# robertvoy/ComfyUI-Distributed

Hardware: NVIDIA H100
Metric: megapixels/sec (higher is better)
Workload: dtype u8

## Files before the change

comfyui-distributed_b200/_native.py:

```python
from __future__ import annotations

import ctypes
import os
from ctypes import POINTER, c_char_p, c_float, c_int, c_int32, c_int64, c_uint32, c_void_p

import numpy as np

HERE = os.path.dirname(os.path.abspath(__file__))
LIB_PATH = os.path.join(HERE, "libusdu_b200.so")

ABI_VERSION = 8
TILE_WORDS = 24
T_X1, T_Y1, T_EW, T_EH, T_PW, T_PH, T_MASK_OFF, T_MASK_PITCH = range(8)
T_TAB_CROP_H, T_TAB_CROP_V, T_TAB_BLEND_H, T_TAB_BLEND_V = 8, 9, 10, 11
T_SUP_X0, T_SUP_Y0, T_SUP_X1, T_SUP_Y1 = 12, 13, 14, 15
T_FULL_X0, T_FULL_Y0, T_FULL_X1, T_FULL_Y1 = 16, 17, 18, 19
TAB_HEADER = 8
PACKED_ROW = 8
FLAG_FAST = 1
FLAG_MMA = 2
FLAG_MMA_KS2 = 4
FLAG_REMOTE_CANVAS = 1 << 24
FILTER_LANCZOS, FILTER_BICUBIC = 0, 1
CROP_ITEM_WORDS = 6
BLEND_ITEM_WORDS = 4
COVER_WORDS = 4
MASK_WORDS = 16
BLOCK_W = 64
BLOCK_H = 32
FAST_BLOCK_W = 128
FAST_BLOCK_H = 32
FAST_TAPS = 7
JOB_WORDS = 32
(J_SRC_A, J_SRC_B, J_LEAD, J_COLS, J_ROWS, J_IX0, J_IY0, J_ROWS_H, J_OX_BASE, J_N_OUT_H, J_ROWS_V, J_OY_BASE, J_N_OUT_V,
 J_DST_X, J_DST_Y, J_OFF_LO, J_OFF_HI, J_ROWS_OUT, J_COLS_OUT, J_CX0, J_CX1, J_CY0, J_CY1, J_FLAGS, J_MPITCH, J_PITCH,
 J_FRAME_LO, J_FRAME_HI, J_NEXT, J_TAPS_H, J_TAPS_V) = range(31)
J_SLOT = 31


class NativeError(RuntimeError):
    pass


_lib = None

_SIGNATURES = {
    "usdu_abi_version": (c_int, []),
    "usdu_last_error": (c_char_p, []),
    "usdu_device_count": (c_int, []),
    "usdu_sm_count": (c_int, []),
    "usdu_resample_ksize": (c_int, [c_int, c_int]),
    "usdu_resample_table_words": (c_int64, [c_int, c_int]),
    "usdu_build_resample_table": (c_int, [c_int, c_int, POINTER(c_int32)]),
    "usdu_build_identity_table": (c_int, [c_int, POINTER(c_int32)]),
    "usdu_filter_ksize": (c_int, [c_int, c_int, c_int]),
    "usdu_filter_table_words": (c_int64, [c_int, c_int, c_int]),
    "usdu_build_filter_table": (c_int, [c_int, c_int, c_int, POINTER(c_int32)]),
    "usdu_nearest_index": (c_int, [c_int, c_int, POINTER(c_int32)]),
    "usdu_table_input_span": (c_int, [POINTER(c_int32), c_int, c_int, POINTER(c_int), POINTER(c_int)]),
    "usdu_box_blur_params": (c_int, [c_float, POINTER(c_int32), POINTER(c_uint32), POINTER(c_uint32)]),
    "usdu_quantize_canvas": (c_int, [c_void_p, c_void_p, c_int, c_int, c_int, c_int64, c_void_p]),
    "usdu_dequantize_canvas": (c_int, [c_void_p, c_void_p, c_int, c_int, c_int, c_int64, c_void_p]),
    "usdu_gather_dequantize": (c_int, [c_void_p, c_void_p, c_int, c_void_p, c_int, c_int, c_int, c_int64, c_void_p]),
    "usdu_level_blend_crop": (c_int, [c_void_p, c_int, c_int, c_int, c_int64, c_void_p, c_void_p, c_void_p, c_int, c_int, c_int, c_void_p, c_int,
                                      c_void_p, c_int, c_int, c_int, c_void_p, c_void_p, c_int, c_void_p, c_int, c_void_p]),
    "usdu_gather_canvas": (c_int, [c_void_p, c_void_p, c_int, c_void_p, c_int, c_int, c_int, c_int64, c_void_p]),
    "usdu_tile_crop_resize_f32": (c_int, [c_void_p, c_int, c_int, c_int, c_void_p, c_void_p, c_int, c_int, c_int, c_void_p, c_int, c_void_p]),
    "usdu_quantize_rows": (c_int, [c_void_p, c_void_p, c_int, c_int, c_int, c_int64, c_int, c_int, c_void_p]),
    "usdu_dequantize_rows": (c_int, [c_void_p, c_void_p, c_int, c_int, c_int, c_int64, c_int, c_int, c_void_p]),
    "usdu_pack_tiles_u8": (c_int, [c_void_p, c_void_p, c_int64, c_void_p]),
    "usdu_unpack_tiles_f32": (c_int, [c_void_p, c_void_p, c_int64, c_void_p]),
    "usdu_t0_denoise": (c_int, [c_void_p, c_void_p, c_void_p, c_int64, c_int64, c_float, c_void_p]),
    "usdu_mask_scratch_bytes": (c_int64, [POINTER(c_int32), c_int]),
    "usdu_build_feather_masks": (c_int, [POINTER(c_int32), c_int, c_void_p, c_void_p, c_void_p]),
    "usdu_plane_resample_u8": (c_int, [c_void_p, c_int, c_int, c_int, c_int64, c_int64, c_void_p, c_int, c_int,
                                       c_void_p, c_int, c_int, c_int, c_int, c_void_p, c_void_p, c_int64, c_int64,
                                       c_void_p]),
    "usdu_plane_pad_fill_u8": (c_int, [c_void_p, c_int, c_int, c_int, c_int64, c_int64, c_int, c_int, c_void_p,
                                       c_void_p, c_void_p, c_int64, c_int64, c_void_p]),
    "usdu_tile_crop_resize": (c_int, [c_void_p, c_int, c_int, c_int, c_int64, c_void_p, c_void_p, c_void_p,
                                      c_int, c_int, c_int, c_void_p, c_int, c_void_p]),
    "usdu_tile_blend": (c_int, [c_void_p, c_int, c_int, c_int, c_int64, c_void_p, c_void_p, c_void_p, c_void_p,
                                c_int, c_void_p, c_int, c_int, c_void_p, c_int, c_int, c_void_p]),
# ... 14 lines not shown
    try:
        h = ctypes.CDLL(LIB_PATH)
    except OSError as e:
        raise NativeError(f"cannot load {LIB_PATH}: {e}") from e
    for name, (res, args) in _SIGNATURES.items():
        try:
            fn = getattr(h, name)
        except AttributeError as e:
            raise NativeError(f"{LIB_PATH} does not export {name}") from e
        fn.restype = res
        fn.argtypes = args
    if h.usdu_abi_version() != ABI_VERSION:
        raise NativeError(f"ABI mismatch: library {h.usdu_abi_version()} != binding {ABI_VERSION}")
    _lib = h
    return h


def _check(status: int, what: str):
    if status != 0:
        msg = lib().usdu_last_error()
        raise NativeError(f"{what} failed ({status}): {msg.decode() if msg else '?'}")


def _i32p(a: np.ndarray):
    assert a.dtype == np.int32 and a.flags["C_CONTIGUOUS"]
    return a.ctypes.data_as(POINTER(c_int32))


def sm_count() -> int:
    n = lib().usdu_sm_count()
    return n if n > 0 else 0


def build_resample_table(in_size: int, out_size: int) -> np.ndarray:
    L = lib()
    words = L.usdu_resample_table_words(in_size, out_size)
    if words < 0:
        _check(int(words), "usdu_resample_table_words")
    tab = np.zeros(int(words), dtype=np.int32)
    _check(L.usdu_build_resample_table(in_size, out_size, _i32p(tab)), "usdu_build_resample_table")
    if tab[4]:
        tab = tab[: int(tab[4]) + out_size * int(tab[6])]
    return np.ascontiguousarray(tab)


def build_filter_table(filt: int, in_size: int, out_size: int) -> np.ndarray:
    L = lib()
    words = L.usdu_filter_table_words(filt, in_size, out_size)
    if words < 0:
        _check(int(words), "usdu_filter_table_words")
    tab = np.zeros(int(words), dtype=np.int32)
    _check(L.usdu_build_filter_table(filt, in_size, out_size, _i32p(tab)), "usdu_build_filter_table")
    return np.ascontiguousarray(tab[: TAB_HEADER + out_size * (2 + int(tab[2]))])


def nearest_index(in_size: int, out_size: int) -> np.ndarray:
    idx = np.zeros(out_size, dtype=np.int32)
    _check(lib().usdu_nearest_index(in_size, out_size, _i32p(idx)), "usdu_nearest_index")
    return idx


def table_input_span(table: np.ndarray, first_out: int, n_out: int):
    a, b = c_int(), c_int()
    _check(lib().usdu_table_input_span(_i32p(table), first_out, n_out, ctypes.byref(a), ctypes.byref(b)),
           "usdu_table_input_span")
    return a.value, b.value
# ... 105 lines not shown
```

comfyui-distributed_b200/csrc/usdu_kernels.cu:

```cuda
#include "usdu_common.cuh"

namespace usdu {

__global__ void __launch_bounds__(kThreads)
quantize_canvas_kernel(const float* __restrict__ img, uint8_t* __restrict__ canvas, int rows, int W3,
                       int64_t pitch, int vec_ok, int H, int y0, int n_rows) {
    const int chunks = (W3 + 15) >> 4;
    const int64_t total = (int64_t)rows * chunks;
    for (int64_t i = (int64_t)blockIdx.x * blockDim.x + threadIdx.x; i < total;
         i += (int64_t)gridDim.x * blockDim.x) {
        const int64_t lrow = i / chunks;
        const int j0 = (int)(i - lrow * chunks) << 4;
        const int64_t fb = lrow / n_rows;
        const int64_t row = fb * H + y0 + (lrow - fb * n_rows);
        const float* src = img + row * W3 + j0;
        uint8_t* dst = canvas + row * pitch + j0;
        if (vec_ok && j0 + 16 <= W3) {
            const float4* s4 = reinterpret_cast<const float4*>(src);
            float4 a = __ldcs(s4), b = __ldcs(s4 + 1), c = __ldcs(s4 + 2), d = __ldcs(s4 + 3);
            uint4 o;
            o.x = quant_u8(a.x) | (quant_u8(a.y) << 8) | (quant_u8(a.z) << 16) | (quant_u8(a.w) << 24);
            o.y = quant_u8(b.x) | (quant_u8(b.y) << 8) | (quant_u8(b.z) << 16) | (quant_u8(b.w) << 24);
            o.z = quant_u8(c.x) | (quant_u8(c.y) << 8) | (quant_u8(c.z) << 16) | (quant_u8(c.w) << 24);
            o.w = quant_u8(d.x) | (quant_u8(d.y) << 8) | (quant_u8(d.z) << 16) | (quant_u8(d.w) << 24);
// ... 415 lines not shown
    const int64_t cap = (int64_t)grid_sms() * 16;
    return (int)(blocks < 1 ? 1 : (blocks > cap ? cap : blocks));
}

static int smem_optin(const void* fn, size_t bytes) {
    if (bytes > 227 * 1024) {
        set_error("kernel needs %zu bytes of shared memory (> 227 KB): patch too large", bytes);
        return USDU_ERR_UNSUPPORTED;
    }
    if (bytes > 48 * 1024) USDU_CUDA(cudaFuncSetAttribute(fn, cudaFuncAttributeMaxDynamicSharedMemorySize, (int)bytes));
    return USDU_OK;
}

}

namespace usdu { namespace fast {
int launch_crop(const uint8_t* canvas, int B, int H, int W, int64_t pitch, const int32_t* tiles, const int32_t* tabs,
                const int32_t* items, int n_items, int patch_w, int patch_h, float* out, cudaStream_t st);
int launch_blend(uint8_t* canvas, int B, int H, int W, int64_t pitch, const int32_t* tiles, const int32_t* tabs,
                 const uint8_t* mask_pool, const int32_t* items, int n_items, const int32_t* cover, int patch_w,
                 int patch_h, const void* src, int src_is_u8, int block_rows, int remote, cudaStream_t st);
} }

namespace usdu { namespace mma {
int launch_crop(const void* canvas, int src_f32, int B, int H, int W, int64_t pitch, const int32_t* tabs, const int32_t* items,
                int n_items, int patch_w, int patch_h, float* out, int two_ksteps, cudaStream_t st);
int launch_blend(uint8_t* canvas, int B, int H, int W, int64_t pitch, const int32_t* tabs, const uint8_t* mask_pool,
                 const int32_t* items, int n_items, int patch_w, int patch_h, const void* src, int src_is_u8, int block_rows,
                 int two_ksteps, cudaStream_t st);
int launch_level(uint8_t* canvas, int B, int H, int W, int64_t pitch, const int32_t* tabs, const uint8_t* mask_pool,
                 const int32_t* bjobs, int n_bheads, int b_patch_w, int b_patch_h, const float* src, int block_rows,
                 const int32_t* cjobs, int n_cjobs, int c_patch_w, int c_patch_h, float* out, const int32_t* expect, int n_slots,
                 int* sync, int two_ksteps, cudaStream_t st);
} }

using namespace usdu;

extern "C" {

int usdu_quantize_rows(const float* img_dev, uint8_t* canvas_dev, int B, int H, int W, int64_t pitch, int y0, int y1,
                       void* stream) {
    USDU_REQUIRE(img_dev && canvas_dev, "usdu_quantize_rows: null pointer");
    USDU_REQUIRE(B > 0 && H > 0 && W > 0, "usdu_quantize_rows: bad shape %dx%dx%d", B, H, W);
    USDU_REQUIRE(0 <= y0 && y0 <= y1 && y1 <= H, "usdu_quantize_rows: bad row range [%d, %d) of %d", y0, y1, H);
    USDU_REQUIRE(pitch >= 3LL * W && pitch % 16 == 0, "usdu_quantize_rows: pitch %lld must be >= 3*W and a multiple of 16", (long long)pitch);
    if (y1 == y0) return USDU_OK;
    const int W3 = W * 3;
    const int vec_ok = (W3 % 4 == 0) && (((uintptr_t)img_dev & 15) == 0) && (((uintptr_t)canvas_dev & 15) == 0);
    const int64_t total = (int64_t)B * (y1 - y0) * ((W3 + 15) / 16);
    const int64_t qblocks = (total + kThreads - 1) / kThreads;
    const int64_t qcap = (int64_t)grid_sms() * 128;
    const int grid = (int)(qblocks < 1 ? 1 : (qblocks > qcap ? qcap : qblocks));
    quantize_canvas_kernel<<<grid, kThreads, 0, (cudaStream_t)stream>>>(img_dev, canvas_dev, B * (y1 - y0), W3, pitch, vec_ok, H, y0, y1 - y0);
    USDU_CUDA(cudaGetLastError());
    return USDU_OK;
}

int usdu_quantize_canvas(const float* img_dev, uint8_t* canvas_dev, int B, int H, int W, int64_t pitch,
                         void* stream) {
    USDU_REQUIRE(H > 0, "usdu_quantize_canvas: bad shape %dx%dx%d", B, H, W);
    return usdu_quantize_rows(img_dev, canvas_dev, B, H, W, pitch, 0, H, stream);
}

int usdu_dequantize_rows(const uint8_t* canvas_dev, float* img_dev, int B, int H, int W, int64_t pitch, int y0, int y1,
                         void* stream) {
    USDU_REQUIRE(img_dev && canvas_dev, "usdu_dequantize_rows: null pointer");
// ... 214 lines not shown
    if (blk_h <= 0 || blk_h > BH) blk_h = BH;
    if (blk_w <= 0 || blk_w > BW) blk_w = BW;
    crop_resize_kernel<<<dim3(n_items, B), kThreads, smem, (cudaStream_t)stream>>>(
        canvas_dev, H, W, pitch, tiles_dev, tabs_dev, items_dev, out_dev, in_pitch, patch_h, blk_w, blk_h);
    USDU_CUDA(cudaGetLastError());
    return USDU_OK;
}

int usdu_tile_crop_resize_f32(const float* image_dev, int B, int H, int W, const int32_t* tabs_dev, const int32_t* items_dev,
                              int n_items, int patch_w, int patch_h, float* out_dev, int flags, void* stream) {
    USDU_REQUIRE(image_dev && tabs_dev && items_dev && out_dev, "usdu_tile_crop_resize_f32: null pointer");
    USDU_REQUIRE(B > 0 && H > 0 && W > 0 && n_items >= 0 && B <= 65535, "usdu_tile_crop_resize_f32: bad shape");
    USDU_REQUIRE(flags & USDU_FLAG_MMA, "usdu_tile_crop_resize_f32: tensor-core job records only (USDU_FLAG_MMA)");
    if (n_items == 0) return USDU_OK;
    return mma::launch_crop(image_dev, 1, B, H, W, (int64_t)W * 3, tabs_dev, items_dev, n_items, patch_w, patch_h, out_dev,
                            (flags & USDU_FLAG_MMA_KS2) ? 1 : 0, (cudaStream_t)stream);
}

int usdu_level_blend_crop(uint8_t* canvas_dev, int B, int H, int W, int64_t pitch, const int32_t* tabs_dev,
                          const uint8_t* mask_pool_dev, const int32_t* bjobs_dev, int n_bheads, int b_patch_w, int b_patch_h,
                          const float* src_dev, int block_rows, const int32_t* cjobs_dev, int n_cjobs, int c_patch_w, int c_patch_h,
                          float* out_dev, const int32_t* expect_dev, int n_slots, int32_t* sync_dev, int flags, void* stream) {
    USDU_REQUIRE(canvas_dev && tabs_dev && mask_pool_dev && bjobs_dev && src_dev && cjobs_dev && out_dev && expect_dev && sync_dev,
                 "usdu_level_blend_crop: null pointer");
    USDU_REQUIRE(B > 0 && B <= 65535 && H > 0 && W > 0 && n_bheads > 0 && n_cjobs > 0 && n_slots > 0, "usdu_level_blend_crop: bad shape");
    USDU_REQUIRE(pitch >= 3LL * W && pitch % 16 == 0, "usdu_level_blend_crop: pitch must be >= 3*W and a multiple of 16");
    USDU_REQUIRE(((uintptr_t)src_dev & 15) == 0, "usdu_level_blend_crop: src must be 16-byte aligned");
    USDU_REQUIRE(flags & USDU_FLAG_MMA, "usdu_level_blend_crop: tensor-core job records only (USDU_FLAG_MMA)");
    return mma::launch_level(canvas_dev, B, H, W, pitch, tabs_dev, mask_pool_dev, bjobs_dev, n_bheads, b_patch_w, b_patch_h, src_dev,
                             block_rows, cjobs_dev, n_cjobs, c_patch_w, c_patch_h, out_dev, expect_dev, n_slots, sync_dev,
                             (flags & USDU_FLAG_MMA_KS2) ? 1 : 0, (cudaStream_t)stream);
}

int usdu_tile_blend(uint8_t* canvas_dev, int B, int H, int W, int64_t pitch, const int32_t* tiles_dev,
                    const int32_t* tabs_dev, const uint8_t* mask_pool_dev, const int32_t* items_dev,
                    int n_items, const int32_t* cover_dev, int patch_w, int patch_h, const void* src_dev,
                    int src_is_u8, int flags, void* stream) {
    USDU_REQUIRE(canvas_dev && tiles_dev && mask_pool_dev && items_dev && src_dev && (cover_dev || (flags & (USDU_FLAG_FAST | USDU_FLAG_MMA))),
                 "usdu_tile_blend: null pointer");
    USDU_REQUIRE(B > 0 && H > 0 && W > 0 && n_items >= 0, "usdu_tile_blend: bad shape");
    USDU_REQUIRE(B <= 65535, "usdu_tile_blend: batch %d exceeds grid.y limit", B);
    USDU_REQUIRE(patch_w > 0 && patch_h > 0, "usdu_tile_blend: patch capacity must be positive");
    if (n_items == 0) return USDU_OK;
    USDU_REQUIRE(pitch >= 3LL * W && pitch % 16 == 0, "usdu_tile_blend: pitch must be >= 3*W and a multiple of 16");
    if (flags & USDU_FLAG_MMA) {
        USDU_REQUIRE(tabs_dev != nullptr, "usdu_tile_blend: tensor-core path needs tables");
        USDU_REQUIRE(((uintptr_t)src_dev & 15) == 0, "usdu_tile_blend: src must be 16-byte aligned");
        return mma::launch_blend(canvas_dev, B, H, W, pitch, tabs_dev, mask_pool_dev, items_dev, n_items, patch_w, patch_h, src_dev,
                                 src_is_u8, (flags >> 8) & 0xFF, (flags & USDU_FLAG_MMA_KS2) ? 1 : 0, (cudaStream_t)stream);
    }
    if (flags & USDU_FLAG_FAST) {
        USDU_REQUIRE(tabs_dev != nullptr, "usdu_tile_blend: fast path needs tables");
        USDU_REQUIRE(((uintptr_t)src_dev & 15) == 0, "usdu_tile_blend: src must be 16-byte aligned");
        return fast::launch_blend(canvas_dev, B, H, W, pitch, tiles_dev, tabs_dev, mask_pool_dev, items_dev, n_items,
                                  cover_dev, patch_w, patch_h, src_dev, src_is_u8, (flags >> 8) & 0xFF,
                                  (flags & USDU_FLAG_REMOTE_CANVAS) ? 1 : 0, (cudaStream_t)stream);
    }
    const int in_pitch = (patch_w * 3 + 15) / 16 * 16;
    const size_t smem = (size_t)BH * BW * 3 + (size_t)patch_h * BW * 3 + (size_t)patch_h * in_pitch;
    const void* fn = src_is_u8 ? (const void*)blend_kernel<true> : (const void*)blend_kernel<false>;
    int s = smem_optin(fn, smem);
    if (s != USDU_OK) return s;
    int blk_h = (flags >> 8) & 0xFF, blk_w = (flags >> 16) & 0xFF;
    if (blk_h <= 0 || blk_h > BH) blk_h = BH;
    if (blk_w <= 0 || blk_w > BW) blk_w = BW;
    if (src_is_u8)
// ... 11 lines not shown
```

comfyui-distributed_b200/csrc/usdu_mma.cu:

```cuda
#include "usdu_common.cuh"
#include "usdu_tma.cuh"
#include <string.h>

namespace usdu {
namespace mma {

constexpr int kT = 256;
constexpr int kOccSmall = 3, kOccLarge = 4;
constexpr int kLargeGridPerSM = 8;
constexpr int BWX = USDU_FAST_BLOCK_W;
constexpr int MIDP = 440;
constexpr int kDBox = BWX * 3 / 2;
constexpr int kBoxB = 256, kBoxR = 48;

__host__ __device__ inline int plane_pitch(int patch_w) { return (patch_w + 31) / 32 * 32 + 16; }
__host__ __device__ inline size_t planes_bytes(int patch_w, int plane_rows) { return (size_t)3 * plane_rows * plane_pitch(patch_w); }
__host__ __device__ inline size_t mid_bytes(int mid_rows) { return (size_t)(mid_rows / 4) * MIDP * 4; }
constexpr size_t kHeadBytes = USDU_JOB_WORDS * 4;

struct JobView {
    const int32_t* j;
    __device__ __forceinline__ int operator[](int i) const { return j[i]; }
    __device__ __forceinline__ int64_t i64(int lo) const { return (int64_t)(uint32_t)j[lo] | ((int64_t)j[lo + 1] << 32); }
};

__device__ __forceinline__ void load_job(int32_t* job_sm, const int32_t* __restrict__ jobs, int idx) {
    if (threadIdx.x < USDU_JOB_WORDS / 4)
        reinterpret_cast<int4*>(job_sm)[threadIdx.x] = __ldg(reinterpret_cast<const int4*>(jobs + (size_t)idx * USDU_JOB_WORDS) + threadIdx.x);
}

__device__ __forceinline__ void mma_uu(int (&d)[4], const uint32_t (&a)[4], uint32_t b0, uint32_t b1) {
    asm("mma.sync.aligned.m16n8k32.row.col.s32.u8.u8.s32 {%0,%1,%2,%3}, {%4,%5,%6,%7}, {%8,%9}, {%0,%1,%2,%3};"
        : "+r"(d[0]), "+r"(d[1]), "+r"(d[2]), "+r"(d[3]) : "r"(a[0]), "r"(a[1]), "r"(a[2]), "r"(a[3]), "r"(b0), "r"(b1));
}
__device__ __forceinline__ void mma_su(int (&d)[4], const uint32_t (&a)[4], uint32_t b0, uint32_t b1) {
    asm("mma.sync.aligned.m16n8k32.row.col.s32.s8.u8.s32 {%0,%1,%2,%3}, {%4,%5,%6,%7}, {%8,%9}, {%0,%1,%2,%3};"
        : "+r"(d[0]), "+r"(d[1]), "+r"(d[2]), "+r"(d[3]) : "r"(a[0]), "r"(a[1]), "r"(a[2]), "r"(a[3]), "r"(b0), "r"(b1));
}

__device__ __forceinline__ int combine(int l0, int l1, int l2) {
    return (l0 + (l1 << 8) + (l2 << 16)) >> kPrecisionBits;
}
// ... 300 lines not shown
            tma::load_3d(raw, &cmap, x, y, b, bar);
            if (two) tma::load_3d(raw + kBoxR * kBoxB, &cmap, x + kBoxB, y, b, bar);
        }
        tma::mbar_wait(bar, 0);
        stage_raw(planes, PB, plane_rows, raw, J[USDU_J_ROWS], J[USDU_J_COLS], sa3 & 15);
    } else if (kSrc == 2) {
        const float* src = reinterpret_cast<const float*>(canvas) + ((int64_t)b * H + J[USDU_J_SRC_B]) * pitch + sa3;
        stage_f32(planes, PB, plane_rows, src, pitch, J[USDU_J_ROWS], J[USDU_J_COLS]);
    } else {
        const uint8_t* src = canvas + ((int64_t)b * H + J[USDU_J_SRC_B]) * pitch + sa3;
        stage_u8(planes, PB, plane_rows, src, pitch, J[USDU_J_ROWS], J[USDU_J_COLS]);
    }
    __syncthreads();
    CropEpilogue epi;
    epi.row_pitch = J[USDU_J_PITCH];
    epi.dst = out + J.i64(USDU_J_OFF_LO) + (int64_t)b * J.i64(USDU_J_FRAME_LO) + (int64_t)J[USDU_J_DST_Y] * epi.row_pitch +
              (int64_t)J[USDU_J_DST_X] * 3;
    epi.ow3 = J[USDU_J_COLS_OUT] * 3;
    epi.rows_out = J[USDU_J_ROWS_OUT];
    both_passes<KSMAX>(planes, mid, tabs, J, PB, plane_rows, J[USDU_J_CY1], epi);
}

struct DTile {
    uint8_t* base;
    int bh;
    __device__ __forceinline__ int strip_off(int strip) const {
        return 4 * strip + (strip >= kDBox / 4 ? bh * kDBox - kDBox : 0);
    }
};

struct BlendOpaque {
    DTile d;
    int nrows;
    uint8_t* rp[2];
    struct Pre {};
    __device__ __forceinline__ void rows(int r0, int r1) {
        rp[0] = (r0 >= 0 && r0 < nrows) ? d.base + r0 * kDBox : nullptr;
        rp[1] = (r1 >= 0 && r1 < nrows) ? d.base + r1 * kDBox : nullptr;
    }
    __device__ __forceinline__ Pre prefetch(int) const { return Pre{}; }
    __device__ __forceinline__ void store(const Pre&, int h, int strip, uint32_t v) {
        if (rp[h] != nullptr) *reinterpret_cast<uint32_t*>(rp[h] + d.strip_off(strip)) = v;
    }
};

struct BlendFeather {
    DTile d;
    const uint8_t* mask;
    int mpitch;
    int cx0, cx1, cy0, cy1;
    uint8_t* rp[2];
    const uint8_t* mp[2];
    struct Pre {
        uint32_t aa[2], ab[2];
        int split;
    };
    __device__ __forceinline__ void rows(int r0, int r1) {
        const bool in0 = r0 >= cy0 && r0 < cy1, in1 = r1 >= cy0 && r1 < cy1;
        rp[0] = in0 ? d.base + r0 * kDBox : nullptr;
        rp[1] = in1 ? d.base + r1 * kDBox : nullptr;
        mp[0] = mask + (int64_t)r0 * mpitch;
        mp[1] = mask + (int64_t)r1 * mpitch;
    }
    __device__ __forceinline__ Pre prefetch(int strip) const {
        const int col = 4 * strip;
        const int pa = col / 3, pb = (col + 3) / 3;
        const bool ina = pa >= cx0 && pa < cx1, inb = pb >= cx0 && pb < cx1;
        Pre p;
        p.split = 3 * pb - col;
#pragma unroll
        for (int h = 0; h < 2; ++h) {
            p.aa[h] = (rp[h] != nullptr && ina) ? (uint32_t)__ldg(mp[h] + pa) : 0u;
            p.ab[h] = (rp[h] != nullptr && inb) ? (uint32_t)__ldg(mp[h] + pb) : 0u;
        }
        return p;
    }
    __device__ __forceinline__ void store(const Pre& p, int h, int strip, uint32_t v) {
        const uint32_t aa = p.aa[h], ab = p.ab[h];
        if ((aa | ab) == 0u) return;
        uint32_t* w = reinterpret_cast<uint32_t*>(rp[h] + d.strip_off(strip));
        if ((aa & ab) == 255u) { *w = v; return; }
        const uint32_t dv = *w;
        uint32_t o = 0;
#pragma unroll
        for (int i = 0; i < 4; ++i) {
            const uint32_t a = i < p.split ? aa : ab;
            o |= composite8((v >> (8 * i)) & 0xFF, (dv >> (8 * i)) & 0xFF, a) << (8 * i);
        }
        *w = o;
    }
};

template <bool kSrcU8, int KSMAX>
__global__ void __launch_bounds__(kT, kOccSmall)
blend_mma_kernel(const int32_t* __restrict__ tabs, const uint8_t* __restrict__ mask_pool, const int32_t* __restrict__ jobs,
                 const void* __restrict__ src_v, int W3, int patch_w, int plane_rows, int mid_rows, int block_rows,
                 const __grid_constant__ CUtensorMap cmap) {
    extern __shared__ __align__(128) uint8_t smem[];
    const size_t dbytes = (size_t)2 * block_rows * kDBox;
    int32_t* job_sm = reinterpret_cast<int32_t*>(smem + dbytes);
    uint64_t* bar = reinterpret_cast<uint64_t*>(smem + dbytes + kHeadBytes);
    uint32_t* mid = reinterpret_cast<uint32_t*>(smem + dbytes + kHeadBytes + 16);
    uint8_t* planes = smem + dbytes + kHeadBytes + 16 + mid_bytes(mid_rows);
    const int PB = plane_pitch(patch_w);
    const int b = blockIdx.y;
    const JobView J{job_sm};
    DTile D{smem, block_rows};
    int idx = blockIdx.x;
    pdl_launch_dependents();
    load_job(job_sm, jobs, idx);
    if (threadIdx.x == 0) tma::mbar_init(bar, 1);
    __syncthreads();
    pdl_wait();
// ... 184 lines not shown
                  (int64_t)J[USDU_J_DST_X] * 3;
        epi.ow3 = J[USDU_J_COLS_OUT] * 3;
        epi.rows_out = J[USDU_J_ROWS_OUT];
        both_passes<KSMAX>(planes, mid, a.tabs, J, PB, a.c_plane_rows, J[USDU_J_CY1], epi);
    }
    __syncthreads();
    if (threadIdx.x == 0) {
        __threadfence();
        s_item = atomicAdd(a.sync + 1, 1);
    }
    __syncthreads();
    if (s_item == total - 1) {
        const int n = 3 + a.n_slots * a.B;
        for (int i = threadIdx.x; i < n; i += kT)
            if (i != 2) a.sync[i] = 0;
        __threadfence();
    }
}

static size_t crop_smem(int patch_w, int plane_rows, int mid_rows, bool use_tma) {
    const size_t region = use_tma ? max(mid_bytes(mid_rows), (size_t)2 * kBoxR * kBoxB) : mid_bytes(mid_rows);
    return region + kHeadBytes + 16 + planes_bytes(patch_w, plane_rows);
}
static size_t blend_smem(int patch_w, int plane_rows, int mid_rows, int block_rows) {
    return (size_t)2 * block_rows * kDBox + kHeadBytes + 16 + planes_bytes(patch_w, plane_rows) + mid_bytes(mid_rows);
}

static int optin(const void* fn, size_t bytes) {
    if (bytes > 227 * 1024) {
        set_error("tensor-core kernel needs %zu bytes of shared memory (> 227 KB)", bytes);
        return USDU_ERR_UNSUPPORTED;
    }
    if (bytes > 48 * 1024) USDU_CUDA(cudaFuncSetAttribute(fn, cudaFuncAttributeMaxDynamicSharedMemorySize, (int)bytes));
    return USDU_OK;
}

static int split_patch_h(int patch_h, int* plane_rows, int* mid_rows, const char* who) {
    *plane_rows = patch_h & 0xFFFF;
    *mid_rows = (patch_h >> 16) & 0xFFFF;
    if (*plane_rows <= 0 || *plane_rows % 8 || *mid_rows < *plane_rows || *mid_rows % 4) {
        set_error("%s: with USDU_FLAG_MMA patch_h carries plane rows (x8) in bits 0..15 and intermediate rows (x4, >= plane rows) "
                  "in bits 16..31; got %d / %d", who, *plane_rows, *mid_rows);
        return USDU_ERR_INVALID;
    }
    return USDU_OK;
}

template <class K, class... Args>
static int launch_one(K kernel, size_t smem, dim3 grid, cudaStream_t st, Args... args) {
    int s = optin((const void*)kernel, smem);
    if (s != USDU_OK) return s;
    USDU_CUDA(launch_pdl(kernel, grid, dim3(kT), smem, st, args...));
    USDU_CUDA(cudaGetLastError());
    return USDU_OK;
}

int launch_crop(const void* canvas, int src_f32, int B, int H, int W, int64_t pitch, const int32_t* tabs, const int32_t* items,
                int n_items, int patch_w, int patch_h, float* out, int two_ksteps, cudaStream_t st) {
    int plane_rows, mid_rows;
    int s = split_patch_h(patch_h, &plane_rows, &mid_rows, "usdu_tile_crop_resize");
    if (s != USDU_OK) return s;
    CUtensorMap cmap;
    memset(&cmap, 0, sizeof(cmap));
    const uint8_t* cv = static_cast<const uint8_t*>(canvas);
    const dim3 grid(n_items, B);
    const int W3 = W * 3;
    const bool large = (int64_t)n_items * B >= (int64_t)kLargeGridPerSM * grid_sms() && !two_ksteps;
#define USDU_CROP_LAUNCH(SRC)                                                                                                                   \
    (two_ksteps ? launch_one(crop_mma_kernel<SRC, 2, kOccSmall>, smem, grid, st, cv, H, pitch, tabs, items, out, patch_w, plane_rows, mid_rows, W3, cmap) \
     : large    ? launch_one(crop_mma_kernel<SRC, 1, kOccLarge>, smem, grid, st, cv, H, pitch, tabs, items, out, patch_w, plane_rows, mid_rows, W3, cmap) \
                : launch_one(crop_mma_kernel<SRC, 1, kOccSmall>, smem, grid, st, cv, H, pitch, tabs, items, out, patch_w, plane_rows, mid_rows, W3, cmap))
    if (src_f32) {
        if (W % 4 != 0 || ((uintptr_t)canvas & 15) != 0) {
            set_error("usdu_tile_crop_resize_f32: the image width must be a multiple of 4 and the image 16-byte aligned");
            return USDU_ERR_UNSUPPORTED;
        }
        const size_t smem = crop_smem(patch_w, plane_rows, mid_rows, false);
        return USDU_CROP_LAUNCH(2);
    }
    bool use_tma = plane_rows <= kBoxR && 12 + patch_w * 3 <= 2 * kBoxB && ((uintptr_t)canvas & 15) == 0;
    if (use_tma) use_tma = tma::encode_u8_3d(&cmap, canvas, (uint64_t)W * 3, (uint64_t)H, (uint64_t)B, (uint64_t)pitch, kBoxB, kBoxR);
    const size_t smem = crop_smem(patch_w, plane_rows, mid_rows, use_tma);
    if (use_tma) return USDU_CROP_LAUNCH(1);
    return USDU_CROP_LAUNCH(0);
#undef USDU_CROP_LAUNCH
}

int launch_blend(uint8_t* canvas, int B, int H, int W, int64_t pitch, const int32_t* tabs, const uint8_t* mask_pool,
                 const int32_t* items, int n_items, int patch_w, int patch_h, const void* src, int src_is_u8, int block_rows,
                 int two_ksteps, cudaStream_t st) {
    if (block_rows != 16 && block_rows != 32) {
        set_error("usdu_tile_blend: the tensor-core path needs a block height of 16 or 32 in flags bits 8..15, got %d", block_rows);
        return USDU_ERR_INVALID;
    }
    int plane_rows, mid_rows;
    int s = split_patch_h(patch_h, &plane_rows, &mid_rows, "usdu_tile_blend");
    if (s != USDU_OK) return s;
    CUtensorMap cmap;
    memset(&cmap, 0, sizeof(cmap));
    if (((uintptr_t)canvas & 15) != 0 ||
// ... 48 lines not shown
```

comfyui-distributed_b200/planner.py:

```python
from __future__ import annotations

import math
import os
from dataclasses import dataclass, field
from typing import Dict, List, Optional, Sequence, Tuple

import numpy as np

from . import _native as nat
from .lru import LruCache


def round_to_multiple(value: int, multiple: int = 8) -> int:
    return round(value / multiple) * multiple


def tile_origins(W: int, H: int, tw: int, th: int) -> List[Tuple[int, int]]:
    cols, rows = math.ceil(W / tw), math.ceil(H / th)
    return [(c * tw, r * th) for r in range(rows) for c in range(cols)]


def _grow(lo: int, hi: int, limit: int, target: int) -> Tuple[int, int]:
    hi = min(hi + (target - (hi - lo)) // 2, limit)
    lo = max(lo - (target - (hi - lo)), 0)
    hi = min(hi + (target - (hi - lo)), limit)
    return lo, hi


@dataclass(frozen=True)
class Tile:
    idx: int
    x: int
    y: int
    x1: int
    y1: int
    x2: int
    y2: int
    pw: int
# ... 355 lines not shown
        best = None
        for k in range(1, world):
            asg = [[] for _ in range(world)]
            for t in self.tiles:
                asg[((t.idx % cols) + k * (t.idx // cols)) % world].append(t.idx)
            if self.conflict_free(asg):
                spread = max(len(a) for a in asg) - min(len(a) for a in asg)
                if best is None or spread < best[0]:
                    best = (spread, asg)
        if best is not None:
            return best[1]
        asg = [[] for _ in range(world)]
        for t in self.tiles:
            asg[t.idx % world].append(t.idx)
        return asg

    def slot_offsets(self, tile_ids: Sequence[int], B: int) -> Tuple[np.ndarray, int]:
        offs = np.zeros(len(tile_ids), dtype=np.int64)
        cur = 0
        for i, tid in enumerate(tile_ids):
            t = self.tiles[tid]
            offs[i] = cur
            cur += B * t.ph * t.pw * 3
        return offs, cur

    def _span_max(self, n_in: int, n_out: int, block: int, aligned: bool) -> int:
        sp = self._tab_span[(n_in, n_out)]
        starts = np.arange(0, n_out, block) if aligned else np.arange(0, n_out)
        ends = np.minimum(starts + block, n_out) - 1
        return int((sp[ends, 1] - sp[starts, 0]).max())

    CTAS_PER_SM = 4
    DEFAULT_SMS = 132

    @classmethod
    def resident_slots(cls) -> int:
        return (nat.sm_count() or cls.DEFAULT_SMS) * cls.CTAS_PER_SM

    def block_shape(self, use_fast: bool, extents: Optional[Sequence[Tuple[int, int]]] = None, frames: int = 1,
                    share: int = 1, mma: bool = False) -> Tuple[int, int]:
        if not use_fast:
            return self._generic_block
        bw = nat.FAST_BLOCK_W
        if not extents:
            return bw, nat.FAST_BLOCK_H
        best = None
        slots = self.resident_slots()
        forced = os.environ.get("USDU_MMA_BH") if mma else None
        for bh in (((int(forced),) if forced else (16, 32)) if mma else (8, 12, 16, 20, 24, 28, 32)):
            n = sum(((w + bw - 1) // bw + 1) * ((h + bh - 1) // bh + 1) for w, h in extents) * frames
            cost = math.ceil(n / max(slots // max(share, 1), 1)) * (bh + 12)
            if best is None or cost < best[0] or (cost == best[0] and bh > best[1]):
                best = (cost, bh)
        return bw, best[1]

    @property
    def _generic_block(self) -> Tuple[int, int]:
        if self._gblock is None:
            bw, bh = nat.BLOCK_W, nat.BLOCK_H
            while True:
                pw_ = max([self._span_max(a, b, bw, False) for (a, b) in self._tab_span] or [bw])
                ph_ = max([self._span_max(a, b, bh, False) for (a, b) in self._tab_span] or [bh])
                smem = nat.BLOCK_H * nat.BLOCK_W * 3 + ph_ * nat.BLOCK_W * 3 + ph_ * ((pw_ * 3 + 15) // 16 * 16)
                if smem <= 200 * 1024 or (bw <= 4 and bh <= 4):
                    break
                if pw_ * bh >= ph_ * bw and bw > 4 or bh <= 4:
                    bw //= 2
                else:
                    bh //= 2
            self._gblock = (bw, bh)
        return self._gblock

    def _crop_block_rows(self, t: Tile, use_fast: bool, bh_max: int) -> int:
        if not use_fast:
            return self._generic_block[1]
        for bh in range(bh_max, 7, -1):
            if self._span_max(t.eh, t.ph, bh, True) <= 40:
                return bh
        return 8

    def kernel_path(self, use_fast=None) -> int:
        path = 2 if use_fast is None else int(use_fast)
        if path >= 2 and not self.mma:
            path = 1
        if path >= 1 and not self.fast:
            path = 0
        return path

    def _mma_crop_rows(self, t: Tile, bh_max: int) -> int:
        key = (t.eh, t.ph)
        for bh in ((32, 16) if bh_max >= 32 else (16,)):
            k0, end, ks = self._tab_k0[key], self._tab_end[key], self._tab_ks[key]
            worst = 0
            for oy0 in range(0, t.ph, bh):
                mv0, mv1 = oy0 // MMA_M, (min(oy0 + bh, t.ph) - 1) // MMA_M
                worst = max(worst, int(end[MMA_M * mv0:min(MMA_M * (mv1 + 1), t.ph)].max() - k0[mv0]))
            if worst <= 48:
                return bh
        return 16

    def crop_worklist(self, tile_ids: Sequence[int], B: int, use_fast: Optional[bool] = None,
                      share: int = 1) -> Tuple[WorkList, np.ndarray, int]:
        path = self.kernel_path(use_fast)
        use_fast = path >= 1
        offs, total = self.slot_offsets(tile_ids, B)
        rows = []
        pw_max = ph_max = 1
        nbytes = 0
        bw, bh_max = self.block_shape(use_fast, [(self.tiles[t].pw - nat.FAST_BLOCK_W, self.tiles[t].ph) for t in tile_ids], B, share,
                                      mma=path == 2)
        for i, tid in enumerate(tile_ids):
            t = self.tiles[tid]
            bh = self._mma_crop_rows(t, bh_max) if path == 2 else self._crop_block_rows(t, use_fast, bh_max)
            ox = np.arange(0, t.pw, bw, dtype=np.int64)
            oy = np.arange(0, t.ph, bh, dtype=np.int64)
            gx, gy = np.meshgrid(ox, oy)
            n = gx.size
            it = np.zeros((n, nat.CROP_ITEM_WORDS), dtype=np.int64)
            it[:, 0], it[:, 1], it[:, 2] = tid, gx.ravel(), gy.ravel()
            it[:, 3], it[:, 4], it[:, 5] = offs[i] & 0xFFFFFFFF, offs[i] >> 32, bh
            rows.append(it)
            pw_max = max(pw_max, self._span_max(t.ew, t.pw, bw, True))
            ph_max = max(ph_max, self._span_max(t.eh, t.ph, bh, True))
            nbytes += t.ew * t.eh * 3 + t.pw * t.ph * 3 * 4
        items = np.concatenate(rows, 0) if rows else np.zeros((0, nat.CROP_ITEM_WORDS), dtype=np.int64)
        if path == 2 and items.shape[0]:
            items, pw_max, ph_max = self._crop_jobs_mma(items)
        elif use_fast and items.shape[0]:
            items = self._crop_jobs(items)
        items = items.astype(np.uint32).view(np.int32) if items.size else items.astype(np.int32)
        ks2 = bool(path == 2 and items.size and (items.reshape(-1, nat.JOB_WORDS)[:, [nat.J_TAPS_H, nat.J_TAPS_V]] > 1).any())
        return WorkList(np.ascontiguousarray(items), None, pw_max, ph_max, nbytes,
                        block_rows=0 if use_fast else bh_max, block_cols=0 if use_fast else bw, path=path, ks2=ks2), offs, total

    def crop_split(self, wl: WorkList, prev_ids: Sequence[int]) -> np.ndarray:
        J = wl.items.reshape(-1, nat.JOB_WORDS).astype(np.int64)
        x0, y0 = J[:, nat.J_SRC_A], J[:, nat.J_SRC_B]
        x1, y1 = x0 + J[:, nat.J_LEAD] + J[:, nat.J_COLS], y0 + J[:, nat.J_ROWS]
        late = np.zeros(J.shape[0], dtype=bool)
        for tid in prev_ids:
            t = self.tiles[tid]
            sx0, sy0, sx1, sy1 = self.support(t)
            if sx1 > sx0 and sy1 > sy0:
# ... 127 lines not shown
            ix1[m] = np.minimum(self._first(key, ox0[m] + nat.FAST_BLOCK_W - 1) + self._tab_taps[key], key[0])
            rows_h[m], taps_h[m] = self._tab_packed[key], self._tab_job_taps[key]
        for key in {(int(a), int(b)) for a, b in zip(eh, ph)}:
            m = (eh == key[0]) & (ph == key[1])
            iy0[m] = self._first(key, oy0[m])
            iy1[m] = np.minimum(self._first(key, oy0[m] + bh[m] - 1) + self._tab_taps[key], key[0])
            rows_v[m], taps_v[m] = self._tab_packed[key], self._tab_job_taps[key]
        J[:, nat.J_TAPS_H], J[:, nat.J_TAPS_V] = taps_h, taps_v
        px_abs = x1 + ix0
        lead = px_abs & 3
        J[:, nat.J_SRC_A], J[:, nat.J_SRC_B], J[:, nat.J_LEAD] = px_abs - lead, y1 + iy0, lead
        J[:, nat.J_COLS], J[:, nat.J_ROWS], J[:, nat.J_IX0], J[:, nat.J_IY0] = ix1 - ix0, iy1 - iy0, ix0, iy0
        J[:, nat.J_ROWS_H], J[:, nat.J_OX_BASE], J[:, nat.J_N_OUT_H] = rows_h, ox0, pw
        J[:, nat.J_ROWS_V], J[:, nat.J_OY_BASE], J[:, nat.J_N_OUT_V] = rows_v, oy0, ph
        J[:, nat.J_DST_X], J[:, nat.J_DST_Y] = ox0, oy0
        J[:, nat.J_OFF_LO], J[:, nat.J_OFF_HI] = items[:, 3], items[:, 4]
        J[:, nat.J_ROWS_OUT] = np.minimum(bh, ph - oy0)
        J[:, nat.J_COLS_OUT] = np.minimum(nat.FAST_BLOCK_W, pw - ox0)
        J[:, nat.J_PITCH] = pw * 3
        frame = ph * pw * 3
        J[:, nat.J_FRAME_LO], J[:, nat.J_FRAME_HI] = frame & 0xFFFFFFFF, frame >> 32
        J[:, nat.J_NEXT] = -1
        return J

    def blend_worklist(self, tile_ids: Sequence[int], offs: np.ndarray, src_bytes_per_elem: int = 4,
                       use_fast: Optional[bool] = None, B: int = 1, part: Optional[Tuple[int, int]] = None,
                       share: int = 1, blocks: Optional[Tuple[np.ndarray, bool]] = None) -> WorkList:
        path = self.kernel_path(use_fast)
        use_fast = path >= 1
        ext = []
        for t in tile_ids:
            sx0, sy0, sx1, sy1 = self.support(self.tiles[t])
            ext.append((sx1 - sx0, sy1 - sy0))
        bw, bh = self.block_shape(use_fast, ext, B, share, mma=path == 2)
        nbx = (self.W + bw - 1) // bw
        nby = (self.H + bh - 1) // bh
        rows = None
        if part is not None:
            i, n = part
            lo_b, hi_b = (nby * i) // n, (nby * (i + 1)) // n
            rows = (min(lo_b * bh, self.H), min(hi_b * bh, self.H))
        sel = None
        if blocks is not None:
            rects, keep = blocks
            hit = np.zeros((nby, nbx), dtype=bool)
            for rx0, ry0, rx1, ry1 in np.asarray(rects, dtype=np.int64).reshape(-1, 4).tolist():
                if rx1 > rx0 and ry1 > ry0:
                    hit[max(ry0, 0) // bh: (min(ry1, self.H) - 1) // bh + 1, max(rx0, 0) // bw: (min(rx1, self.W) - 1) // bw + 1] = True
            sel = (hit if keep else ~hit).ravel()
        keys, tids, seq = [], [], []
        pw_max = ph_max = 1
        nbytes = 0
        for s, tid in enumerate(tile_ids):
            t = self.tiles[tid]
            sx0, sy0, sx1, sy1 = self.support(t)
            if sx1 <= sx0 or sy1 <= sy0:
                continue
            X0, Y0, X1, Y1 = t.x1 + sx0, t.y1 + sy0, t.x1 + sx1, t.y1 + sy1
            gx = np.arange(X0 // bw, (X1 - 1) // bw + 1, dtype=np.int64)
            gy = np.arange(Y0 // bh, (Y1 - 1) // bh + 1, dtype=np.int64)
            if part is not None:
                gy = gy[(gy >= lo_b) & (gy < hi_b)]
                if gy.size == 0:
                    continue
            k = (gy[:, None] * nbx + gx[None, :]).ravel()
            n_all = k.size
            if sel is not None:
# ... 117 lines not shown
```

include/usdu_b200.h:

```cpp
#ifndef USDU_B200_H
#define USDU_B200_H

#include <stddef.h>
#include <stdint.h>

#ifdef __cplusplus
extern "C" {
#endif
#if defined(__GNUC__)
#pragma GCC visibility push(default)
#endif

#define USDU_ABI_VERSION 8

typedef enum usdu_status {
    USDU_OK = 0,
    USDU_ERR_INVALID = -1,
    USDU_ERR_CUDA = -2,
    USDU_ERR_UNSUPPORTED = -3
} usdu_status;

#define USDU_TILE_WORDS 24
#define USDU_T_X1 0
#define USDU_T_Y1 1
// ... 42 lines not shown
#define USDU_J_OY_BASE 11
#define USDU_J_N_OUT_V 12
#define USDU_J_DST_X 13
#define USDU_J_DST_Y 14
#define USDU_J_OFF_LO 15
#define USDU_J_OFF_HI 16
#define USDU_J_ROWS_OUT 17
#define USDU_J_COLS_OUT 18
#define USDU_J_CX0 19
#define USDU_J_CX1 20
#define USDU_J_CY0 21
#define USDU_J_CY1 22
#define USDU_J_FLAGS 23
#define USDU_J_MPITCH 24
#define USDU_J_PITCH 25
#define USDU_J_FRAME_LO 26
#define USDU_J_FRAME_HI 27
#define USDU_J_NEXT 28
#define USDU_J_SLOT 31
#define USDU_J_TAPS_H 29
#define USDU_J_TAPS_V 30

#define USDU_MASK_WORDS 16

#define USDU_BLOCK_W 64
#define USDU_BLOCK_H 32
#define USDU_FAST_BLOCK_W 128
#define USDU_FAST_BLOCK_H 32

int usdu_abi_version(void);
const char* usdu_last_error(void);
int usdu_device_count(void);
int usdu_sm_count(void);

int usdu_resample_ksize(int in_size, int out_size);
int64_t usdu_resample_table_words(int in_size, int out_size);
int usdu_build_resample_table(int in_size, int out_size, int32_t* table);
#define USDU_FILTER_LANCZOS 0
#define USDU_FILTER_BICUBIC 1
int usdu_filter_ksize(int filter, int in_size, int out_size);
int64_t usdu_filter_table_words(int filter, int in_size, int out_size);
int usdu_build_filter_table(int filter, int in_size, int out_size, int32_t* table);
int usdu_nearest_index(int in_size, int out_size, int32_t* index_host);
int usdu_build_identity_table(int size, int32_t* table);
int usdu_box_blur_params(float radius, int32_t* rad, uint32_t* ww, uint32_t* fw);

#define USDU_FLAG_FAST 1
#define USDU_FLAG_MMA 2
#define USDU_FLAG_MMA_KS2 4
#define USDU_FLAG_BLOCK_ROWS(n) ((n) << 8)
#define USDU_FLAG_BLOCK_COLS(n) ((n) << 16)
#define USDU_FLAG_REMOTE_CANVAS (1 << 24)
int usdu_quantize_canvas(const float* img_dev, uint8_t* canvas_dev, int B, int H, int W,
                         int64_t pitch, void* stream);
int usdu_dequantize_canvas(const uint8_t* canvas_dev, float* img_dev, int B, int H, int W,
                           int64_t pitch, void* stream);
int usdu_quantize_rows(const float* img_dev, uint8_t* canvas_dev, int B, int H, int W, int64_t pitch,
                       int y0, int y1, void* stream);
int usdu_dequantize_rows(const uint8_t* canvas_dev, float* img_dev, int B, int H, int W, int64_t pitch,
                         int y0, int y1, void* stream);
#define USDU_MAX_SLABS 16
int usdu_gather_dequantize(const uint8_t* const* slab_canvas_dev, const int32_t* slab_rows, int n_slabs,
                           float* img_dev, int B, int H, int W, int64_t pitch, void* stream);
int usdu_gather_canvas(const uint8_t* const* slab_canvas_dev, const int32_t* slab_rows, int n_slabs,
                       uint8_t* canvas_dev, int B, int H, int W, int64_t pitch, void* stream);
int usdu_pack_tiles_u8(const float* src_dev, uint8_t* dst_dev, int64_t n, void* stream);
// ... 47 lines not shown
```

Before: 20760.

## Drive block-height planning from queried MMA kernel occupancy

```diff
diff --git a/comfyui-distributed_b200/_native.py b/comfyui-distributed_b200/_native.py
--- a/comfyui-distributed_b200/_native.py
+++ b/comfyui-distributed_b200/_native.py
@@ -21,6 +21,7 @@
 FLAG_MMA = 2
 FLAG_MMA_KS2 = 4
 FLAG_REMOTE_CANVAS = 1 << 24
+MMA_BLEND_F32, MMA_BLEND_U8, MMA_CROP = 0, 1, 2
 FILTER_LANCZOS, FILTER_BICUBIC = 0, 1
 CROP_ITEM_WORDS = 6
 BLEND_ITEM_WORDS = 4
@@ -49,6 +50,7 @@
     "usdu_last_error": (c_char_p, []),
     "usdu_device_count": (c_int, []),
     "usdu_sm_count": (c_int, []),
+    "usdu_mma_ctas_per_sm": (c_int, [c_int, c_int, c_int64, c_int64]),
     "usdu_resample_ksize": (c_int, [c_int, c_int]),
     "usdu_resample_table_words": (c_int64, [c_int, c_int]),
     "usdu_build_resample_table": (c_int, [c_int, c_int, POINTER(c_int32)]),
@@ -129,6 +131,13 @@
     return n if n > 0 else 0
 
 
+def mma_ctas_per_sm(kind: int, grid_ctas: int, smem_bytes: int, two_ksteps: bool = False) -> int:
+    n = lib().usdu_mma_ctas_per_sm(kind, FLAG_MMA_KS2 if two_ksteps else 0, int(grid_ctas), int(smem_bytes))
+    if n < 0:
+        _check(n, "usdu_mma_ctas_per_sm")
+    return n
+
+
 def build_resample_table(in_size: int, out_size: int) -> np.ndarray:
     L = lib()
     words = L.usdu_resample_table_words(in_size, out_size)
diff --git a/comfyui-distributed_b200/csrc/usdu_kernels.cu b/comfyui-distributed_b200/csrc/usdu_kernels.cu
--- a/comfyui-distributed_b200/csrc/usdu_kernels.cu
+++ b/comfyui-distributed_b200/csrc/usdu_kernels.cu
@@ -471,6 +471,7 @@
                  const int32_t* bjobs, int n_bheads, int b_patch_w, int b_patch_h, const float* src, int block_rows,
                  const int32_t* cjobs, int n_cjobs, int c_patch_w, int c_patch_h, float* out, const int32_t* expect, int n_slots,
                  int* sync, int two_ksteps, cudaStream_t st);
+int ctas_per_sm(int kind, int two_ksteps, int64_t grid_ctas, int64_t smem);
 } }
 
 using namespace usdu;
@@ -751,6 +752,11 @@
                              (flags & USDU_FLAG_MMA_KS2) ? 1 : 0, (cudaStream_t)stream);
 }
 
+int usdu_mma_ctas_per_sm(int kind, int flags, int64_t grid_ctas, int64_t smem_bytes) {
+    USDU_REQUIRE(grid_ctas >= 0 && smem_bytes >= 0, "usdu_mma_ctas_per_sm: negative grid or shared-memory size");
+    return mma::ctas_per_sm(kind, (flags & USDU_FLAG_MMA_KS2) ? 1 : 0, grid_ctas, smem_bytes);
+}
+
 int usdu_tile_blend(uint8_t* canvas_dev, int B, int H, int W, int64_t pitch, const int32_t* tiles_dev,
                     const int32_t* tabs_dev, const uint8_t* mask_pool_dev, const int32_t* items_dev,
                     int n_items, const int32_t* cover_dev, int patch_w, int patch_h, const void* src_dev,
diff --git a/comfyui-distributed_b200/csrc/usdu_mma.cu b/comfyui-distributed_b200/csrc/usdu_mma.cu
--- a/comfyui-distributed_b200/csrc/usdu_mma.cu
+++ b/comfyui-distributed_b200/csrc/usdu_mma.cu
@@ -7,7 +7,7 @@
 
 constexpr int kT = 256;
 constexpr int kOccSmall = 3, kOccLarge = 4;
-constexpr int kLargeGridPerSM = 8;
+constexpr int kLargeGridPerSM = kOccSmall;
 constexpr int BWX = USDU_FAST_BLOCK_W;
 constexpr int MIDP = 440;
 constexpr int kDBox = BWX * 3 / 2;
@@ -374,15 +374,15 @@
 struct BlendOpaque {
     DTile d;
     int nrows;
-    uint8_t* rp[2];
+    int ro[2];
     struct Pre {};
     __device__ __forceinline__ void rows(int r0, int r1) {
-        rp[0] = (r0 >= 0 && r0 < nrows) ? d.base + r0 * kDBox : nullptr;
-        rp[1] = (r1 >= 0 && r1 < nrows) ? d.base + r1 * kDBox : nullptr;
+        ro[0] = (r0 >= 0 && r0 < nrows) ? r0 * kDBox : -1;
+        ro[1] = (r1 >= 0 && r1 < nrows) ? r1 * kDBox : -1;
     }
     __device__ __forceinline__ Pre prefetch(int) const { return Pre{}; }
     __device__ __forceinline__ void store(const Pre&, int h, int strip, uint32_t v) {
-        if (rp[h] != nullptr) *reinterpret_cast<uint32_t*>(rp[h] + d.strip_off(strip)) = v;
+        if (ro[h] >= 0) *reinterpret_cast<uint32_t*>(d.base + ro[h] + d.strip_off(strip)) = v;
     }
 };
 
@@ -391,18 +391,18 @@
     const uint8_t* mask;
     int mpitch;
     int cx0, cx1, cy0, cy1;
-    uint8_t* rp[2];
-    const uint8_t* mp[2];
+    int ro[2];
+    int mo[2];
     struct Pre {
         uint32_t aa[2], ab[2];
         int split;
     };
     __device__ __forceinline__ void rows(int r0, int r1) {
         const bool in0 = r0 >= cy0 && r0 < cy1, in1 = r1 >= cy0 && r1 < cy1;
-        rp[0] = in0 ? d.base + r0 * kDBox : nullptr;
-        rp[1] = in1 ? d.base + r1 * kDBox : nullptr;
-        mp[0] = mask + (int64_t)r0 * mpitch;
-        mp[1] = mask + (int64_t)r1 * mpitch;
+        ro[0] = in0 ? r0 * kDBox : -1;
+        ro[1] = in1 ? r1 * kDBox : -1;
+        mo[0] = r0 * mpitch;
+        mo[1] = r1 * mpitch;
     }
     __device__ __forceinline__ Pre prefetch(int strip) const {
         const int col = 4 * strip;
@@ -412,15 +412,15 @@
         p.split = 3 * pb - col;
 #pragma unroll
         for (int h = 0; h < 2; ++h) {
-            p.aa[h] = (rp[h] != nullptr && ina) ? (uint32_t)__ldg(mp[h] + pa) : 0u;
-            p.ab[h] = (rp[h] != nullptr && inb) ? (uint32_t)__ldg(mp[h] + pb) : 0u;
+            p.aa[h] = (ro[h] >= 0 && ina) ? (uint32_t)__ldg(mask + mo[h] + pa) : 0u;
+            p.ab[h] = (ro[h] >= 0 && inb) ? (uint32_t)__ldg(mask + mo[h] + pb) : 0u;
         }
         return p;
     }
     __device__ __forceinline__ void store(const Pre& p, int h, int strip, uint32_t v) {
         const uint32_t aa = p.aa[h], ab = p.ab[h];
         if ((aa | ab) == 0u) return;
-        uint32_t* w = reinterpret_cast<uint32_t*>(rp[h] + d.strip_off(strip));
+        uint32_t* w = reinterpret_cast<uint32_t*>(d.base + ro[h] + d.strip_off(strip));
         if ((aa & ab) == 255u) { *w = v; return; }
         const uint32_t dv = *w;
         uint32_t o = 0;
@@ -671,7 +671,41 @@
         return USDU_ERR_UNSUPPORTED;
     }
     if (bytes > 48 * 1024) USDU_CUDA(cudaFuncSetAttribute(fn, cudaFuncAttributeMaxDynamicSharedMemorySize, (int)bytes));
+    USDU_CUDA(cudaFuncSetAttribute(fn, cudaFuncAttributePreferredSharedMemoryCarveout, cudaSharedmemCarveoutMaxShared));
     return USDU_OK;
+}
+
+static bool crop_large_grid(int64_t ctas, int two_ksteps, int sms) {
+    return ctas >= (int64_t)kLargeGridPerSM * sms && !two_ksteps;
+}
+constexpr int kDefaultSms = 132;
+
+template <class K>
+static int resident(K kernel, int compiled, int64_t smem) {
+    if (smem > 227 * 1024) return 0;
+    if (sm_count() <= 0) return compiled;
+    int s = optin((const void*)kernel, (size_t)smem);
+    if (s != USDU_OK) return s;
+    int n = 0;
+    USDU_CUDA(cudaOccupancyMaxActiveBlocksPerMultiprocessor(&n, kernel, kT, (size_t)smem));
+    return n;
+}
+
+int ctas_per_sm(int kind, int two_ksteps, int64_t grid_ctas, int64_t smem) {
+    switch (kind) {
+    case USDU_MMA_BLEND_F32:
+        return two_ksteps ? resident(blend_mma_kernel<false, 2>, kOccSmall, smem) : resident(blend_mma_kernel<false, 1>, kOccSmall, smem);
+    case USDU_MMA_BLEND_U8:
+        return two_ksteps ? resident(blend_mma_kernel<true, 2>, kOccSmall, smem) : resident(blend_mma_kernel<true, 1>, kOccSmall, smem);
+    case USDU_MMA_CROP: {
+        const int n = sm_count();
+        if (two_ksteps) return resident(crop_mma_kernel<1, 2, kOccSmall>, kOccSmall, smem);
+        return crop_large_grid(grid_ctas, 0, n > 0 ? n : kDefaultSms) ? resident(crop_mma_kernel<1, 1, kOccLarge>, kOccLarge, smem)
+                                                                      : resident(crop_mma_kernel<1, 1, kOccSmall>, kOccSmall, smem);
+    }
+    }
+    set_error("usdu_mma_ctas_per_sm: unknown kernel kind %d", kind);
+    return USDU_ERR_INVALID;
 }
 
 static int split_patch_h(int patch_h, int* plane_rows, int* mid_rows, const char* who) {
@@ -704,7 +738,7 @@
     const uint8_t* cv = static_cast<const uint8_t*>(canvas);
     const dim3 grid(n_items, B);
     const int W3 = W * 3;
-    const bool large = (int64_t)n_items * B >= (int64_t)kLargeGridPerSM * grid_sms() && !two_ksteps;
+    const bool large = crop_large_grid((int64_t)n_items * B, two_ksteps, grid_sms());
 #define USDU_CROP_LAUNCH(SRC)                                                                                                                   \
     (two_ksteps ? launch_one(crop_mma_kernel<SRC, 2, kOccSmall>, smem, grid, st, cv, H, pitch, tabs, items, out, patch_w, plane_rows, mid_rows, W3, cmap) \
      : large    ? launch_one(crop_mma_kernel<SRC, 1, kOccLarge>, smem, grid, st, cv, H, pitch, tabs, items, out, patch_w, plane_rows, mid_rows, W3, cmap) \
diff --git a/comfyui-distributed_b200/planner.py b/comfyui-distributed_b200/planner.py
--- a/comfyui-distributed_b200/planner.py
+++ b/comfyui-distributed_b200/planner.py
@@ -3,7 +3,7 @@
 import math
 import os
 from dataclasses import dataclass, field
-from typing import Dict, List, Optional, Sequence, Tuple
+from typing import Callable, Dict, List, Optional, Sequence, Tuple
 
 import numpy as np
 
@@ -425,23 +425,50 @@
 
     CTAS_PER_SM = 4
     DEFAULT_SMS = 132
+    MMA_CROP_SMEM = 2 * 48 * 256 + nat.JOB_WORDS * 4 + 16 + 3 * 48 * ((166 + 31) // 32 * 32 + 16)
 
     @classmethod
-    def resident_slots(cls) -> int:
-        return (nat.sm_count() or cls.DEFAULT_SMS) * cls.CTAS_PER_SM
+    def resident_slots(cls, ctas_per_sm: Optional[int] = None) -> int:
+        return (nat.sm_count() or cls.DEFAULT_SMS) * max(cls.CTAS_PER_SM if ctas_per_sm is None else ctas_per_sm, 1)
+
+    def _crop_footprint(self, tile_ids: Sequence[int]) -> Tuple[int, bool]:
+        ks2 = any(self._tab_ks[(t.ew, t.pw)] > 1 or self._tab_ks[(t.eh, t.ph)] > 1 for t in (self.tiles[i] for i in tile_ids))
+        return self.MMA_CROP_SMEM, ks2
+
+    def _blend_footprint(self, tile_ids: Sequence[int], bw: int, bh: int) -> Tuple[int, bool]:
+        pw_ = rows = need_h = 1
+        ks2 = False
+        for tid in tile_ids:
+            t = self.tiles[tid]
+            sx0, sy0, sx1, sy1 = self.support(t)
+            if sx1 <= sx0 or sy1 <= sy0:
+                continue
+            X0, Y0, X1, Y1 = t.x1 + sx0, t.y1 + sy0, t.x1 + sx1, t.y1 + sy1
+            ox = np.arange(X0 // bw, (X1 - 1) // bw + 1, dtype=np.int64) * bw - t.x1
+            oy = np.arange(Y0 // bh, (Y1 - 1) // bh + 1, dtype=np.int64) * bh - t.y1
+            _, ks_h, _, cnt, need = self._mma_axis((t.pw, t.ew), ox, np.full(ox.size, bw))
+            pw_ = max(pw_, int(((cnt + 3) & ~3).max()), int(need.max()))
+            _, ks_v, _, cnt, need = self._mma_axis((t.ph, t.eh), oy, np.full(oy.size, bh))
+            rows, need_h = max(rows, int(cnt.max())), max(need_h, int(need.max()))
+            ks2 = ks2 or ks_h > 1 or ks_v > 1
+        ph_ = self._mma_patch_h(np.array([rows]), np.array([need_h]), pw_)
+        plane_rows, mid_rows = ph_ & 0xFFFF, ph_ >> 16
+        return (2 * bh * nat.FAST_BLOCK_W * 3 // 2 + nat.JOB_WORDS * 4 + 16 + 3 * plane_rows * ((pw_ + 31) // 32 * 32 + 16) +
+                mid_rows // 4 * 440 * 4), ks2
 
     def block_shape(self, use_fast: bool, extents: Optional[Sequence[Tuple[int, int]]] = None, frames: int = 1,
-                    share: int = 1, mma: bool = False) -> Tuple[int, int]:
+                    share: int = 1, mma: bool = False, kind: int = nat.MMA_CROP,
+                    footprint: Optional[Callable[[int], Tuple[int, bool]]] = None) -> Tuple[int, int]:
         if not use_fast:
             return self._generic_block
         bw = nat.FAST_BLOCK_W
         if not extents:
             return bw, nat.FAST_BLOCK_H
         best = None
-        slots = self.resident_slots()
         forced = os.environ.get("USDU_MMA_BH") if mma else None
         for bh in (((int(forced),) if forced else (16, 32)) if mma else (8, 12, 16, 20, 24, 28, 32)):
             n = sum(((w + bw - 1) // bw + 1) * ((h + bh - 1) // bh + 1) for w, h in extents) * frames
+            slots = self.resident_slots(nat.mma_ctas_per_sm(kind, n, *(footprint(bh) if footprint else (0, False))) if mma else None)
             cost = math.ceil(n / max(slots // max(share, 1), 1)) * (bh + 12)
             if best is None or cost < best[0] or (cost == best[0] and bh > best[1]):
                 best = (cost, bh)
@@ -501,7 +528,7 @@
         pw_max = ph_max = 1
         nbytes = 0
         bw, bh_max = self.block_shape(use_fast, [(self.tiles[t].pw - nat.FAST_BLOCK_W, self.tiles[t].ph) for t in tile_ids], B, share,
-                                      mma=path == 2)
+                                      mma=path == 2, kind=nat.MMA_CROP, footprint=lambda bh: self._crop_footprint(tile_ids))
         for i, tid in enumerate(tile_ids):
             t = self.tiles[tid]
             bh = self._mma_crop_rows(t, bh_max) if path == 2 else self._crop_block_rows(t, use_fast, bh_max)
@@ -695,7 +722,9 @@
         for t in tile_ids:
             sx0, sy0, sx1, sy1 = self.support(self.tiles[t])
             ext.append((sx1 - sx0, sy1 - sy0))
-        bw, bh = self.block_shape(use_fast, ext, B, share, mma=path == 2)
+        bw, bh = self.block_shape(use_fast, ext, B, share, mma=path == 2,
+                                  kind=nat.MMA_BLEND_U8 if src_bytes_per_elem == 1 else nat.MMA_BLEND_F32,
+                                  footprint=lambda bh_: self._blend_footprint(tile_ids, nat.FAST_BLOCK_W, bh_))
         nbx = (self.W + bw - 1) // bw
         nby = (self.H + bh - 1) // bh
         rows = None
diff --git a/include/usdu_b200.h b/include/usdu_b200.h
--- a/include/usdu_b200.h
+++ b/include/usdu_b200.h
@@ -98,6 +98,10 @@
 const char* usdu_last_error(void);
 int usdu_device_count(void);
 int usdu_sm_count(void);
+#define USDU_MMA_BLEND_F32 0
+#define USDU_MMA_BLEND_U8 1
+#define USDU_MMA_CROP 2
+int usdu_mma_ctas_per_sm(int kind, int flags, int64_t grid_ctas, int64_t smem_bytes);
 
 int usdu_resample_ksize(int in_size, int out_size);
 int64_t usdu_resample_table_words(int in_size, int out_size);
```

After: 21200 (median of 6 runs). 1.02x the previous value.
